# tirtho109/parallel_AMG

Hardware: AMD Instinct MI355X
Metric: V-cycle iters/sec + fine-SpMV HBM GB/s, 3D Poisson 128M dofs at 1/2/4/8 GPU (higher is better)
Workload: dtype f64; 1 GPU; poisson3d 512^3 fp64, SA-AMG V(1,1) weighted-Jacobi, 1 part(s); n=134217728, nnz_fine=937951232, levels=6, max_coarse=1000, parallelism=row-slab partition p1

## Files before the change

### include/pamg.h

```cpp
#ifndef PAMG_H
#define PAMG_H

#include <stdint.h>

#ifdef __cplusplus
extern "C" {
#endif

#define PAMG_OK 0
#define PAMG_E_ARG (-1)
#define PAMG_E_HIP (-2)
#define PAMG_E_RCCL (-3)
#define PAMG_E_OVERFLOW (-4)
#define PAMG_E_SETUP (-5)
#define PAMG_E_STATE (-6)
#define PAMG_E_NOMEM (-7)

typedef struct pamg_ctx pamg_ctx;
typedef struct pamg_plan pamg_plan;
typedef struct pamg_vec pamg_vec;
typedef struct pamg_mat pamg_mat;
typedef struct pamg_hier pamg_hier;
typedef struct pamg_hcsr pamg_hcsr;

// ... 42 lines not shown
int pamg_vec_download(pamg_ctx* ctx, const pamg_vec* v, double* own);
int pamg_vec_download_ghosts(pamg_ctx* ctx, const pamg_vec* v, double* ghost);
int pamg_vec_device_ptr(pamg_vec* v, double** dptr);
int pamg_vec_fill(pamg_ctx* ctx, pamg_vec* v, double value);
int pamg_vec_copy(pamg_ctx* ctx, const pamg_vec* src, pamg_vec* dst);
int pamg_vec_axpby(pamg_ctx* ctx, double a, const pamg_vec* x, double b, pamg_vec* y);
int pamg_vec_dot(pamg_ctx* ctx, const pamg_vec* x, const pamg_vec* y, double* out);
int pamg_vec_nrm2(pamg_ctx* ctx, const pamg_vec* x, double* out);
int pamg_exchange(pamg_ctx* ctx, const pamg_plan* plan, pamg_vec* x);
int pamg_exchange_begin(pamg_ctx* ctx, pamg_plan* plan, pamg_vec* x);
int pamg_exchange_end(pamg_ctx* ctx, pamg_plan* plan, pamg_vec* x);

int pamg_mat_upload(pamg_ctx* ctx, int64_t nrows, int64_t ncols_local, const int64_t* rowptr,
                    const void* col, int col_is_64, const double* val, int index_base,
                    const pamg_plan* col_plan, pamg_mat** out);
int pamg_mat_upload_perm(pamg_ctx* ctx, int64_t nrows, int64_t ncols_local, const int64_t* rowptr,
                         const void* col, int col_is_64, const double* val, int index_base,
                         const pamg_plan* col_plan, const int64_t* row_perm,
                         const int64_t* col_perm, pamg_mat** out);
int pamg_mat_destroy(pamg_mat* A);
int pamg_mat_info(const pamg_mat* A, int64_t* nrows, int64_t* ncols_local, int64_t* nnz);
int pamg_mat_stream_bytes(const pamg_mat* A, int64_t* bytes);
int pamg_mat_layout(const pamg_mat* A, int set, int out[10]);

int pamg_spmv(pamg_ctx* ctx, const pamg_mat* A, pamg_vec* x, pamg_vec* y);
int pamg_residual(pamg_ctx* ctx, const pamg_mat* A, pamg_vec* x, const pamg_vec* b,
                  pamg_vec* r, double* nrm2);
int pamg_jacobi(pamg_ctx* ctx, const pamg_mat* A, pamg_vec* x, const pamg_vec* b,
                pamg_vec* tmp, double omega, int nsweeps);
int pamg_jacobi_residual(pamg_ctx* ctx, const pamg_mat* A, pamg_vec* x, const pamg_vec* b,
                         pamg_vec* t, pamg_vec* r, double omega, int* fused);

int pamg_hier_create(pamg_ctx* ctx, int nlevels, pamg_mat* const* A, pamg_mat* const* P,
                     pamg_mat* const* R, const double* omega, int64_t n_coarse,
                     const double* ainv_colmajor, int rep_level, const int64_t* rep_offsets,
                     pamg_hier** out);
int pamg_hier_destroy(pamg_hier* H);
int pamg_hier_set_graph(pamg_hier* H, int enable);
int pamg_hier_set_sweeps(pamg_hier* H, int nu1, int nu2);
int pamg_hier_set_perm(pamg_hier* H, int64_t n, const int64_t* perm);
int pamg_hier_graph_state(const pamg_hier* H, int* enabled, int* captured, int* failed);
int pamg_vcycle(pamg_ctx* ctx, pamg_hier* H, pamg_vec* x, const pamg_vec* b, int ncycles,
                double* res_hist);
int pamg_vcycle_async(pamg_ctx* ctx, pamg_hier* H, pamg_vec* x, const pamg_vec* b, int ncycles);
int pamg_pcg(pamg_ctx* ctx, pamg_hier* H, pamg_vec* x, const pamg_vec* b, double rtol,
             int maxit, int* iters, double* res_hist);
// ... 51 lines not shown
```

### parallel_amg_amd/_lib.py

```python
from __future__ import annotations

import ctypes as C
import os

_HERE = os.path.dirname(os.path.abspath(__file__))
LIB_PATH = os.environ.get("PAMG_LIB") or os.path.join(_HERE, "libpamg.so")

PAMG_OK = 0
ERRORS = {-1: "PAMG_E_ARG", -2: "PAMG_E_HIP", -3: "PAMG_E_RCCL", -4: "PAMG_E_OVERFLOW",
          -5: "PAMG_E_SETUP", -6: "PAMG_E_STATE", -7: "PAMG_E_NOMEM"}


class PamgError(RuntimeError):
    def __init__(self, code, fn, msg):
        super().__init__(f"{fn} -> {ERRORS.get(code, code)}: {msg}")
        self.code = code


vp = C.c_void_p
i32, i64, dbl = C.c_int, C.c_int64, C.c_double
pvp = C.POINTER(C.c_void_p)
pi64 = C.POINTER(C.c_int64)
pdbl = C.POINTER(C.c_double)
pi32 = C.POINTER(C.c_int32)
# ... 27 lines not shown
    "pamg_plan_set_tag": [vp, i64],
    "pamg_plan_destroy": [vp],
    "pamg_vec_create": [vp, i64, i64, pvp],
    "pamg_vec_destroy": [vp],
    "pamg_vec_size": [vp, pi64, pi64],
    "pamg_vec_upload": [vp, vp, vp],
    "pamg_vec_download": [vp, vp, vp],
    "pamg_vec_download_ghosts": [vp, vp, vp],
    "pamg_vec_device_ptr": [vp, pvp],
    "pamg_vec_fill": [vp, vp, dbl],
    "pamg_vec_copy": [vp, vp, vp],
    "pamg_vec_axpby": [vp, dbl, vp, dbl, vp],
    "pamg_vec_dot": [vp, vp, vp, pdbl],
    "pamg_vec_nrm2": [vp, vp, pdbl],
    "pamg_exchange": [vp, vp, vp],
    "pamg_exchange_begin": [vp, vp, vp],
    "pamg_exchange_end": [vp, vp, vp],
    "pamg_mat_upload": [vp, i64, i64, vp, vp, i32, vp, i32, vp, pvp],
    "pamg_mat_upload_perm": [vp, i64, i64, vp, vp, i32, vp, i32, vp, vp, vp, pvp],
    "pamg_mat_destroy": [vp],
    "pamg_mat_info": [vp, pi64, pi64, pi64],
    "pamg_mat_stream_bytes": [vp, pi64],
    "pamg_mat_layout": [vp, i32, C.POINTER(C.c_int)],
    "pamg_spmv": [vp, vp, vp, vp],
    "pamg_residual": [vp, vp, vp, vp, vp, pdbl],
    "pamg_jacobi": [vp, vp, vp, vp, vp, dbl, i32],
    "pamg_jacobi_residual": [vp, vp, vp, vp, vp, vp, dbl, pi32],
    "pamg_hier_create": [vp, i32, vp, vp, vp, vp, i64, vp, i32, vp, pvp],
    "pamg_hier_destroy": [vp],
    "pamg_hier_set_graph": [vp, i32],
    "pamg_hier_set_sweeps": [vp, i32, i32],
    "pamg_hier_set_perm": [vp, i64, vp],
    "pamg_hier_graph_state": [vp, C.POINTER(C.c_int), C.POINTER(C.c_int), C.POINTER(C.c_int)],
    "pamg_vcycle": [vp, vp, vp, vp, i32, vp],
    "pamg_vcycle_async": [vp, vp, vp, vp, i32],
    "pamg_pcg": [vp, vp, vp, vp, dbl, i32, C.POINTER(C.c_int), vp],
    "pamg_hier_profile": [vp, i32],
    "pamg_hier_profile_read": [vp, vp],
    "pamg_bench_rowop": [vp, vp, i32, vp, vp, vp, dbl, i32, pdbl],
    "pamg_hier_bench_chain": [vp, vp, vp, i32, pdbl],
    "pamg_set_option": [C.c_char_p, i64],
    "pamg_get_option": [C.c_char_p, pi64],
    "pamg_hcsr_create": [i64, i64, i64, pvp],
    "pamg_hcsr_destroy": [vp],
    "pamg_hcsr_info": [vp, pi64, pi64, pi64],
    "pamg_hcsr_data": [vp, C.POINTER(pi64), C.POINTER(pi32), C.POINTER(pdbl)],
# ... 50 lines not shown
    for key, sym in (("hip", "hipStreamCreateWithFlags"), ("rccl", "ncclCommInitRank")):
        try:
            addr = C.cast(getattr(L, sym), C.c_void_p).value
        except AttributeError:
            continue
        info = _DlInfo()
        if addr and dladdr(addr, C.byref(info)) and info.dli_fname:
            out[key] = os.path.realpath(info.dli_fname.decode())
    return out


def call(name, *args):
    L = lib()
    rc = getattr(L, name)(*args)
    if rc != PAMG_OK:
        msg = L.pamg_last_error().decode(errors="replace")
        raise PamgError(rc, name, msg)
    return rc


def layout_of(M, part_set: int = 0) -> dict:
    out = (C.c_int * 10)()
    call("pamg_mat_layout", M.handle, part_set, out)
    return {"c24": bool(out[0]), "vd": bool(out[1]), "rl8": bool(out[2]), "cd": int(out[3]),
            "cd_offsets": int(out[4]), "tm": bool(out[5]), "tm_rs": int(out[6]),
            "tile_nnz": int(out[7]), "tiles": int(out[8]), "anchored": bool(out[9] & 1), "per_tile": bool(out[9] & 2),
            "x_stage": bool(out[9] & 4), "sym": bool(out[9] & 8), "sym_rows": 2 if out[9] & 16 else 1,
            "jr_fused": bool(out[9] & 32), "tm_vd": bool(out[9] & 64), "sym_vd": bool(out[9] & 128),
            "ell": bool(out[9] & 512), "pnc": bool(out[9] & 1024),
            "rpat": bool(out[9] & 2048), "pnc_compact": bool(out[9] & 4096),
            "ell_pair": bool(out[9] & 8192)}


def last_error() -> str:
    return lib().pamg_last_error().decode(errors="replace")


def ptr(a):
    return C.c_void_p(a.ctypes.data) if a is not None and a.size else None
```

### parallel_amg_amd/csrc/kernels.hip

```cpp

#include "pamg_device.h"

namespace pamg {
namespace {

__device__ __forceinline__ int wave_incl_scan(int v) {
    const int lane = threadIdx.x & 63, rl = lane & 15;
    int t;
    t = __builtin_amdgcn_mov_dpp(v, 0x111, 0xf, 0xf, false);
    if (rl >= 1) v += t;
    t = __builtin_amdgcn_mov_dpp(v, 0x112, 0xf, 0xf, false);
    if (rl >= 2) v += t;
    t = __builtin_amdgcn_mov_dpp(v, 0x114, 0xf, 0xf, false);
    if (rl >= 4) v += t;
    t = __builtin_amdgcn_mov_dpp(v, 0x118, 0xf, 0xf, false);
    if (rl >= 8) v += t;
    t = __builtin_amdgcn_mov_dpp(v, 0x142, 0xf, 0xf, false);
    if (lane & 16) v += t;
    t = __builtin_amdgcn_mov_dpp(v, 0x143, 0xf, 0xf, false);
    if (lane >= 32) v += t;
    return v;
}

template <int OP>
// ... 1477 lines not shown
            const bool ok = 4 * q + e < L;
            const double p = vv[e] * xv[e];
            const double t = s + p;
            s = ok ? t : s;
            if constexpr (OP == OP_JACOBI) dg = ok && of[e] == 0 ? vv[e] : dg;
        }
    }
    double out;
    if constexpr (OP == OP_SPMV) {
        out = s;
    } else if constexpr (OP == OP_RESID) {
        out = pb - s;
    } else if constexpr (OP == OP_JACOBI) {
        const double u = pb - s;
        const double v = omega * u;
        const double w = v / dg;
        out = px + w;
    } else {
        out = py + s;
    }
    if (in) y[i] = out;
}

template <int OP, int U>
__global__ __launch_bounds__(kEllGroup) void k_rows_rpat(int nrows, const int* __restrict__ gorder,
                                                         const int* __restrict__ anc, const uint8_t* __restrict__ pid,
                                                         const int2* __restrict__ pmeta, int npat,
                                                         const uint32_t* __restrict__ pent, int nent,
                                                         const double* __restrict__ vtab, int nval, int ngroups,
                                                         const double* __restrict__ x, const double* __restrict__ b,
                                                         double* __restrict__ y, double omega) {
    __shared__ uint32_t le[kRpatEnt];
    __shared__ int2 lm[kRpatMax];
    __shared__ double lv[256];
    const int per = (ngroups + 7) / 8;
    const int gi = (blockIdx.x & 7) * per + (blockIdx.x >> 3);
    if (gi >= ngroups) return;
    const int g = gorder ? gorder[gi] : gi;
    const int tid = threadIdx.x;
    const int i = g * kEllGroup + tid;
    const int ic = i < nrows ? i : nrows - 1;
    const int p = i < nrows ? (int)pid[i] : kRpatSkip;
    const int a = anc[ic];
    double pb = 0.0, px = 0.0, py = 0.0;
    if constexpr (OP == OP_RESID || OP == OP_JACOBI) pb = b[ic];
    if constexpr (OP == OP_JACOBI) px = x[ic];
// ... 525 lines not shown

template <int OP>
void launch_rpat(const pamg_mat& A, const double* x, const double* b, double* y, double omega, hipStream_t s) {
    const RpatSet& R = A.rpat;
    const int grid = (int)((R.ngroups + 7) / 8 * 8);
    auto go = [&](auto kern) {
        kern<<<grid, kEllGroup, 0, s>>>((int)A.nrows, R.d_gorder, R.d_anc, R.d_pid, R.d_pmeta, R.npat, R.d_pent, R.nent,
                                        R.d_vtab, R.nval, (int)R.ngroups, x, b, y, omega);
    };
    go(k_rows_rpat<OP, 8>);
}

template <int OP>
void launch_rows_op(const pamg_mat& A, const TileSet& ts, const double* x, const double* b,
                    double* y, double omega, hipStream_t s) {
    if (ts.sym) launch_sym<OP>(A, x, b, y, omega, s);
    if (ts.ell) {
        const EllSet& E = A.ell;
        const int grid = (int)((E.ngroups + 7) / 8 * 8);
        auto go = [&](auto kern) {
            kern<<<grid, kEllGroup, 0, s>>>((int)A.nrows, E.d_gorder, E.d_anc, E.d_smeta, E.d_ci, E.d_vi, E.d_len,
                                            E.d_gmeta, E.d_otab, E.d_vtab, (int)E.ngroups, x, b, y, omega);
        };
        if (E.d_anc) {
            if (E.paired) go(k_rows_ell<OP, true, true>);
            else go(k_rows_ell<OP, true, false>);
        } else {
            if (E.paired) go(k_rows_ell<OP, false, true>);
            else go(k_rows_ell<OP, false, false>);
        }
    }
    if (ts.pnc) launch_pnc<OP>(A, x, b, y, omega, s);
    if (ts.rpat) launch_rpat<OP>(A, x, b, y, omega, s);
    if (ts.n_short > 0) {
        if (ts.tile_nnz == 1024) launch_tile<OP, 1024>(A, ts, x, b, y, omega, s);
        else if (ts.tile_nnz == 4096) launch_tile<OP, 4096>(A, ts, x, b, y, omega, s);
        else launch_tile<OP, 2048>(A, ts, x, b, y, omega, s);
    }
    if (ts.n_long > 0)
        k_rows_long<OP><<<ts.n_long, kBlock, 0, s>>>(ts.d_long, A.d_rowptr, A.d_col, A.d_val, x,
                                                     b, y, omega);
}
}

void launch_sym_tb(const pamg_mat& A, const TbArgs& ta, hipStream_t s) {
    SymDia sd = A.sym;
    TbGeom& g = sd.tb;
// ... 106 lines not shown
```

### parallel_amg_amd/csrc/pamg_device.h

```cpp
#pragma once

#include <hip/hip_runtime.h>
#include <rccl/rccl.h>

#include <atomic>
#include <cstdint>
#include <array>
#include <mutex>
#include <vector>

#include "pamg_common.h"

namespace pamg {

constexpr int kBlock = 256;
constexpr int kTileRows = 256;

constexpr int kXsMaxClusters = 12;
constexpr int kTmSmallTab = 128;
constexpr int kXsCap = 1088;
constexpr int kXsIoff = 128;
constexpr int kXsGap = 48;
struct XStage {
    int ncl = 0, stride = 0, zix = -1, ncols = 0;
// ... 56 lines not shown
    int col_dict = 1;
    int tile_major = 1;
    int col_dict_tile = 1;
    int tm_tile_dicts = 1;
    int band_pct = 100;
    int band_pct_restrict = 50;
    int x_stage = 1;
    int col_dict_anchor = 1;
    int poison_ghosts = 0;
    int sym_dia = 1;
    int sym_rows = 2;
    int jr_fuse = 1;
    int symd_chunks = 2;
    int chain_store_x = 0;
    int tb_xfast = 1;
    int sym_zm = 1;
    int zm_chunks = 0;
    int ell = 1;
    int ell_min_rows = 65536;
    int ell_restrict = 1;
    int ell_yblock = 16;
    int rpat = 1;
    int ell_pair = 1;
    int pnc_compact = 1;
    int pnc = 1;
    int sym_vd = 1;
};

constexpr int kSymMaxU = 7;
constexpr int kSymVdMax = 64;
struct TbGeom {
    int nx = 0, ny = 0, nz = 0;
    int tiles_x = 0, tiles_y = 0;
    int zchunks = 1, zlen = 0;
    int zlo = 0, zhi = 0;
    int xfast = 0;
};
constexpr int kEllW = 64;
constexpr int kEllGroup = 256;
constexpr int kEllSkip = 255;
struct EllSet {
    int64_t nslices = 0, ngroups = 0;
    int2* d_smeta = nullptr;
    uint32_t* d_ci = nullptr;
    uint32_t* d_vi = nullptr;
    uint8_t* d_len = nullptr;
    int4* d_gmeta = nullptr;
    int* d_otab = nullptr;
    double* d_vtab = nullptr;
    int* d_anc = nullptr;
    int* d_gorder = nullptr;
    int64_t words = 0, otab_n = 0, vtab_n = 0;
    bool paired = false;
};

constexpr int kPncPatMax = 1024, kPncValMax = 128, kPncMaxLen = 7;
constexpr int kPncSkip = kPncPatMax - 1;
constexpr int kPncCombMax = 1024;
constexpr int kPncCombSkip = 0xffff;
struct PncSet {
    int nx = 0, ny = 0, nz = 0;
    int* d_anc = nullptr;
    uint2* d_rec = nullptr;
    uint16_t* d_cid = nullptr;
    uint64_t* d_pvals = nullptr;
    uint32_t* d_ptab = nullptr;
    double* d_vtab = nullptr;
    int npat = 0, nval = 0;
    int grid = 0;
};

constexpr int kRpatMax = 255, kRpatEnt = 4096, kRpatMaxLen = 128;
constexpr int kRpatSkip = 255;
struct RpatSet {
    int64_t ngroups = 0;
    int* d_anc = nullptr;
// ... 134 lines not shown
```

### parallel_amg_amd/csrc/runtime.hip

```cpp
#include <dlfcn.h>

#include <algorithm>
#include <array>
#include <atomic>
#include <functional>
#include <chrono>
#include <condition_variable>
#include <mutex>
#include <cstdio>
#include <cstdlib>
#include <cstring>
#include <map>
#include <memory>
#include <mutex>
#include <string>
#include <thread>
#include <vector>

#include "pamg_device.h"

using pamg::fail;

pamg::Options& pamg::options() {
    static Options o;
    return o;
}

#define HIPC(expr)                                                                    \
// ... 1108 lines not shown
            const int64_t gnx = gr[1], gny = gr[2], gM = gr[1] * gr[2];
            std::vector<int64_t> key(ng);
            par_for(ng, [&](int64_t a, int64_t b) {
                for (int64_t g = a; g < b; ++g) {
                    const int64_t c = anc[g * kEllGroup];
                    const int64_t y = (c / gnx) % gny, z = c / gM;
                    key[g] = ((y / yb) << 40) | (z << 20) | y;
                }
            });
            const int64_t per = (ng + 7) / 8;
            std::vector<int> order(ng);
            for (int64_t g = 0; g < ng; ++g) order[g] = (int)g;
            for (int64_t e = 0; e < 8; ++e) {
                const int64_t lo = std::min(ng, e * per), hi = std::min(ng, (e + 1) * per);
                std::stable_sort(order.begin() + lo, order.begin() + hi, [&](int p, int q) { return key[p] < key[q]; });
            }
            CHECK(dalloc(d_order, ng));
            CHECK(h2d(ctx, *d_order, order.data(), sizeof(int) * ng));
            break;
        }
    return PAMG_OK;
}

int build_ell(pamg_mat* A, const PtrVec& rp, const IdxVec& ci, const double* val,
              bool anchored, const std::vector<int>& inner) {
    using pamg::kEllGroup;
    using pamg::kEllSkip;
    using pamg::kEllW;
    const int64_t n = A->nrows;
    std::vector<char> in_set;
    if ((int64_t)inner.size() != n) {
        in_set.assign(n, 0);
        for (int i : inner) in_set[i] = 1;
    }
    auto member = [&](int64_t i) { return in_set.empty() || in_set[i]; };
    auto base_of = [&](int64_t i) -> int { return anchored ? (rp[i + 1] > rp[i] ? ci[rp[i]] : 0) : (int)i; };
    const int64_t ns = (n + kEllW - 1) / kEllW, ng = (n + kEllGroup - 1) / kEllGroup;
    std::vector<int> slen(ns, 0);
    std::atomic<bool> ok{true};
    par_for(ns, [&](int64_t a, int64_t b) {
        for (int64_t q = a; q < b; ++q) {
            int m = 0;
            for (int64_t i = q * kEllW; i < std::min(n, (q + 1) * kEllW); ++i)
                if (member(i)) m = std::max<int>(m, (int)(rp[i + 1] - rp[i]));
            if (m >= kEllSkip) ok = false;
            slen[q] = m;
        }
    });
    if (!ok) return PAMG_OK;
    std::vector<int2> smeta(ns);
    int64_t words = 0;
    for (int64_t q = 0; q < ns; ++q) {
        smeta[q] = make_int2((int)words, slen[q]);
        words += (int64_t)kEllW * ((slen[q] + 3) / 4);
        if (words >= INT32_MAX) return PAMG_OK;
    }
    std::vector<std::vector<int>> goff(ng);
    std::vector<std::vector<uint64_t>> gval(ng);
    std::vector<uint32_t> cw(words + 1, 0u), vw;
    std::vector<uint8_t> len(n + kVecPad, 0);
    bool paired = pamg::options().ell_pair != 0;
    if (paired) {
        std::atomic<bool> fits{true};
        par_for(ng, [&](int64_t a, int64_t b) {
            constexpr int kSlots = 1024;
            std::vector<int> pid(kSlots), pstamp(kSlots, -1), pkey_o(kSlots);
            std::vector<uint64_t> pkey_v(kSlots);
            std::vector<int> o;
            std::vector<uint64_t> v;
            for (int64_t g = a; g < b && fits; ++g) {
                const int stamp = (int)(g - a);
                o.clear();
                v.clear();
                const int64_t r1 = std::min(n, (g + 1) * kEllGroup);
                for (int64_t i = g * kEllGroup; i < r1 && fits; ++i) {
                    if (!member(i)) {
                        len[i] = (uint8_t)kEllSkip;
                        continue;
// ... 481 lines not shown
    R = pamg::RpatSet{};
}

void free_pnc(pamg::PncSet& P) {
    dfree(P.d_anc);
    dfree(P.d_rec);
    dfree(P.d_cid);
    dfree(P.d_pvals);
    dfree(P.d_ptab);
    dfree(P.d_vtab);
    P = pamg::PncSet{};
}

void free_ell(pamg::EllSet& E) {
    dfree(E.d_gorder);
    dfree(E.d_smeta);
    dfree(E.d_ci);
    dfree(E.d_vi);
    dfree(E.d_len);
    dfree(E.d_gmeta);
    dfree(E.d_otab);
    dfree(E.d_vtab);
    dfree(E.d_anc);
    E = pamg::EllSet{};
}

void free_tiles(pamg::TileSet& ts) {
    dfree(ts.d_short);
    dfree(ts.d_long);
    dfree(ts.d_base);
    dfree(ts.d_vtab);
    dfree(ts.d_ctab);
    ts.cd = ts.ctab_n = 0;
    dfree(ts.d_tm_val);
    dfree(ts.d_tm_cidx);
    dfree(ts.d_tm_clo);
    dfree(ts.d_tm_chi);
    dfree(ts.d_tm_rlen);
    dfree(ts.d_tm_anc);
    dfree(ts.d_tm_vidx);
    dfree(ts.d_tm_vtab);
    ts.tm_vt = 0;
    dfree(ts.d_abase);
    ts.anc = ts.pt = ts.xs = false;
    ts.tm = false;
    ts.tm_rs = 0;
// ... 1253 lines not shown
        CHECK(build_col_dicts(A.get(), rp, ci, t_in, t_bd, &idx8));
        tr.mark("col dicts");
        CHECK(build_tile_major(A.get(), n_own_cols, rp, ci, val, t_in, t_bd, lo, hi, idx8));
        tr.mark("tile-major");
    }
    if (A->interior.rl8 || A->boundary.rl8) {
        std::vector<uint8_t> rl(nrows + kVecPad, 0);
        par_for(nrows, [&](int64_t a, int64_t b) {
            for (int64_t i = a; i < b; ++i) rl[i] = (uint8_t)std::min<int64_t>(255, rp[i + 1] - rp[i]);
        });
        CHECK(dalloc(&A->d_rlen, nrows + kVecPad));
        CHECK(h2d(ctx, A->d_rlen, rl.data(), rl.size()));
    }
    if (!vidx.empty()) {
        CHECK(dalloc(&A->d_vidx, (int64_t)vidx.size()));
        CHECK(h2d(ctx, A->d_vidx, vidx.data(), vidx.size()));
    }
    A->stream_bytes = 4;
    if (A->interior.sym)
        A->stream_bytes += A->sym.vd_n ? nrows + (int64_t)A->sym.vd_n * (8 * (A->sym.nu + 1) + 4)
                                       : nrows * (A->sym.mask_bytes + 8 + 8 * (int64_t)A->sym.nu);
    if (A->interior.ell)
        A->stream_bytes += (A->ell.paired ? 4 : 8) * A->ell.words + nrows + 8 * A->ell.nslices + 16 * A->ell.ngroups + 4 * A->ell.otab_n +
                           8 * A->ell.vtab_n + (A->ell.d_anc ? 4 * nrows : 0);
    if (A->interior.pnc)
        A->stream_bytes += (A->pnc.d_cid ? 6 : 12) * nrows + (A->pnc.d_cid ? 12 : 4) * A->pnc.npat + 8 * A->pnc.nval;
    if (A->interior.rpat) A->stream_bytes += 5 * nrows + 8 * A->rpat.npat + 4 * A->rpat.nent + 8 * A->rpat.nval;
    for (const pamg::TileSet* t : {&A->interior, &A->boundary}) {
        if (t->sym || t->ell || t->pnc || t->rpat) continue;
        const int64_t ns = t->n_short, nz = t->nnz_short;
        int64_t b = 8 * (int64_t)t->n_long + 12 * t->nnz_long;
        const bool base = t->c24 && !t->cd;
        if (t->tm) {
            const int64_t tn = t->tile_nnz;
            const int64_t rowb = t->tm_rs;
            const int64_t valb = t->tm_vt ? tn + 8 * (int64_t)t->tm_vt : 8 * tn;
            b += ns * (rowb * (t->anc ? 5 : 1) + valb + (t->cd ? t->cd * tn / 8 : 3 * tn) + 16 + (base ? 4 : 0)) +
                 (t->cd ? 4 * t->ctab_n * (t->pt ? ns : 1) : 0);
        } else {
            b += (t->rl8 ? 1 : 4) * t->rows_short;
            b += t->cd ? (t->cd * nz + 7) / 8 + 4 * t->ctab_n * (t->pt ? ns : 1) : (t->c24 ? 3 : 4) * nz;
            if (t->pt && t->anc) b += 2 * t->rows_short + 4 * ns;
            b += t->vd ? nz / 2 + 128 * ns : 8 * nz;
            b += (16 + (base ? 4 : 0)) * ns;
        }
        A->stream_bytes += b;
    }
// ... 126 lines not shown
    out[5] = t.tm;
    out[6] = t.tm_rs;
    out[7] = t.tile_nnz;
    out[8] = t.n_short;
    out[9] = (t.anc ? 1 : 0) | (t.pt ? 2 : 0) | (t.xs ? 4 : 0) | (t.sym ? 8 : 0) | (t.sym && A->sym.rpl == 2 ? 16 : 0) |
             (t.sym && (A->sym.tb_ok || A->sym.tb_part) ? 32 : 0) | (t.tm && t.tm_vt ? 64 : 0) |
             (t.sym && A->sym.vd_n ? 128 : 0) | (t.ell ? 512 : 0) | (t.pnc ? 1024 : 0) | (t.rpat ? 2048 : 0) |
             (t.pnc && A->pnc.d_cid ? 4096 : 0) | (t.ell && A->ell.paired ? 8192 : 0);
    if (t.ell) out[8] = (int)A->ell.ngroups;
    if (t.rpat) {
        out[3] = A->rpat.nval;
        out[4] = A->rpat.npat;
        out[8] = (int)A->rpat.ngroups;
    }
    if (t.pnc) {
        out[3] = A->pnc.nval;
        out[4] = A->pnc.npat;
        out[8] = A->pnc.grid;
    }
    if (t.sym) {
        out[4] = A->sym.nu;
        out[8] = A->sym.nbands * 8 * A->sym.eighth;
    }
    return PAMG_OK;
}

static int check_vec_for(const pamg_mat* A, const pamg_vec* x, const char* who) {
    const int64_t need_ghost = A->plan ? A->plan->n_ghost : 0;
    const int64_t own = A->plan ? A->plan->n_own : A->ncols;
    if (x->n_own != own || x->n_ghost < need_ghost)
        return fail(PAMG_E_ARG, "%s: input vector (%lld own, %lld ghost) does not fit the matrix columns (%lld own, %lld ghost)",
                    who, (long long)x->n_own, (long long)x->n_ghost, (long long)own, (long long)need_ghost);
    return PAMG_OK;
}

int pamg_spmv(pamg_ctx* ctx, const pamg_mat* A, pamg_vec* x, pamg_vec* y) {
    if (!ctx || !A || !x || !y) return fail(PAMG_E_ARG, "spmv: NULL");
    CHECK(check_vec_for(A, x, "spmv"));
    if (y->n_own != A->nrows) return fail(PAMG_E_ARG, "spmv: output size mismatch");
    if (x == y) return fail(PAMG_E_ARG, "spmv: x and y must differ");
    CHECK(set_device(ctx));
    CHECK(apply(ctx, A, pamg::OP_SPMV, x->d, nullptr, y->d, 0.0));
    HIPC(hipStreamSynchronize(ctx->s_comp));
    return PAMG_OK;
}

// ... 584 lines not shown
    else if (k == "value_dict" && value >= 0 && value <= 2) o.value_dict = (int)value;
    else if (k == "col_dict" && (value == 0 || value == 1)) o.col_dict = (int)value;
    else if (k == "tile_major" && value >= 0 && value <= 2) o.tile_major = (int)value;
    else if (k == "col_dict_anchor" && (value == 0 || value == 1)) o.col_dict_anchor = (int)value;
    else if (k == "col_dict_tile" && (value == 0 || value == 1)) o.col_dict_tile = (int)value;
    else if (k == "x_stage" && (value == 0 || value == 1)) o.x_stage = (int)value;
    else if (k == "band_pct" && value >= 1 && value <= 10000) o.band_pct = (int)value;
    else if (k == "band_pct_restrict" && value >= 1 && value <= 10000) o.band_pct_restrict = (int)value;
    else if (k == "long_tiles_min" && value >= 1 && value <= 255) o.long_tiles_min = (int)value;
    else if (k == "tm_tile_dicts" && (value == 0 || value == 1)) o.tm_tile_dicts = (int)value;
    else if (k == "sym_dia" && (value == 0 || value == 1)) o.sym_dia = (int)value;
    else if (k == "sym_rows" && (value == 1 || value == 2)) o.sym_rows = (int)value;
    else if (k == "jr_fuse" && (value == 0 || value == 1)) o.jr_fuse = (int)value;
    else if (k == "sym_vd" && (value == 0 || value == 1)) o.sym_vd = (int)value;
    else if (k == "symd_chunks" && (value == 1 || value == 2 || value == 4)) o.symd_chunks = (int)value;
    else if (k == "sym_zm" && (value == 0 || value == 1)) o.sym_zm = (int)value;
    else if (k == "tb_xfast" && (value == 0 || value == 1)) o.tb_xfast = (int)value;
    else if (k == "ell" && (value == 0 || value == 1)) o.ell = (int)value;
    else if (k == "ell_restrict" && (value == 0 || value == 1)) o.ell_restrict = (int)value;
    else if (k == "pnc" && (value == 0 || value == 1)) o.pnc = (int)value;
    else if (k == "rpat" && (value == 0 || value == 1)) o.rpat = (int)value;
    else if (k == "pnc_compact" && (value == 0 || value == 1)) o.pnc_compact = (int)value;
    else if (k == "ell_pair" && (value == 0 || value == 1)) o.ell_pair = (int)value;
    else if (k == "ell_yblock" && value >= 0 && value <= 65536) o.ell_yblock = (int)value;
    else if (k == "ell_min_rows" && value >= 0 && value <= INT32_MAX) o.ell_min_rows = (int)value;
    else if (k == "zm_chunks" && value >= 0 && value <= 4096) o.zm_chunks = (int)value;
    else if (k == "chain_store_x" && (value == 0 || value == 1)) o.chain_store_x = (int)value;
    else return fail(PAMG_E_ARG, "set_option: unknown key or bad value: %s=%lld", key, (long long)value);
    return PAMG_OK;
}

int pamg_get_option(const char* key, int64_t* value) {
    if (!key || !value) return fail(PAMG_E_ARG, "get_option: bad args");
    const auto& o = pamg::options();
    const std::string k(key);
    if (k == "tile_nnz") *value = o.tile_nnz;
    else if (k == "tile_order") *value = o.tile_order;
    else if (k == "long_tiles") *value = o.long_tiles;
    else if (k == "row_len8") *value = o.row_len8;
    else if (k == "poison_ghosts") *value = o.poison_ghosts;
    else if (k == "col24") *value = o.col24;
    else if (k == "value_dict") *value = o.value_dict;
    else if (k == "col_dict") *value = o.col_dict;
    else if (k == "tile_major") *value = o.tile_major;
    else if (k == "col_dict_anchor") *value = o.col_dict_anchor;
    else if (k == "col_dict_tile") *value = o.col_dict_tile;
    else if (k == "x_stage") *value = o.x_stage;
    else if (k == "band_pct") *value = o.band_pct;
    else if (k == "band_pct_restrict") *value = o.band_pct_restrict;
    else if (k == "long_tiles_min") *value = o.long_tiles_min;
    else if (k == "tm_tile_dicts") *value = o.tm_tile_dicts;
    else if (k == "sym_dia") *value = o.sym_dia;
    else if (k == "sym_rows") *value = o.sym_rows;
    else if (k == "jr_fuse") *value = o.jr_fuse;
    else if (k == "sym_vd") *value = o.sym_vd;
    else if (k == "symd_chunks") *value = o.symd_chunks;
    else if (k == "sym_zm") *value = o.sym_zm;
    else if (k == "tb_xfast") *value = o.tb_xfast;
    else if (k == "ell") *value = o.ell;
    else if (k == "ell_restrict") *value = o.ell_restrict;
    else if (k == "pnc") *value = o.pnc;
    else if (k == "rpat") *value = o.rpat;
    else if (k == "pnc_compact") *value = o.pnc_compact;
    else if (k == "ell_pair") *value = o.ell_pair;
    else if (k == "ell_yblock") *value = o.ell_yblock;
    else if (k == "ell_min_rows") *value = o.ell_min_rows;
    else if (k == "zm_chunks") *value = o.zm_chunks;
    else if (k == "chain_store_x") *value = o.chain_store_x;
    else return fail(PAMG_E_ARG, "get_option: unknown key %s", key);
    return PAMG_OK;
}

int pamg_hier_bench_chain(pamg_hier* H, pamg_vec* x, const pamg_vec* b, int reps, double* avg_ms) {
    if (!H || !x || !b || reps < 1 || !avg_ms) return fail(PAMG_E_ARG, "hier_bench_chain: bad args");
    if (!pipe_ok(H, 2, false)) return fail(PAMG_E_STATE, "hier_bench_chain: the hierarchy does not run the cross-cycle pipeline");
    pamg_ctx* ctx = H->ctx;
    CHECK(check_vec_for(H->A[0], x, "hier_bench_chain"));
    CHECK(set_device(ctx));
    if (!H->u0) {
        const int64_t n = H->nown[0] + (H->A[0]->plan ? H->A[0]->plan->n_ghost : 0) + kVecPad;
        CHECK(dalloc(&H->u0, n));
        CHECK(dzero(H->ctx, H->u0, sizeof(double) * n));
    }
    hipEvent_t e0, e1;
    HIPC(hipEventCreate(&e0));
    HIPC(hipEventCreate(&e1));
    hipStream_t s = ctx->s_comp;
// ... 75 lines not shown
```

Baseline: 218.9 V-cycles/s.

## Add windowed ELL kernel staging x into LDS via async global_load_lds

Adds an ELL variant that groups four row slices by shared (offset,value) pairs and column coupling, then stages the contiguous x window each group touches into LDS with global_load_lds before the row sweep. Rows then read x from LDS using 16-bit local offsets instead of gathering from global memory. The aim is to cut redundant and uncoalesced x gathers in the ELL row kernels (spmv, residual, jacobi, prolong), which mostly hit coarse levels. In exchange it adds a heavy host-side grouping pass, extra metadata streams (chunks, lof, dpos), and LDS pressure that may lower occupancy; it is gated on window size and share thresholds.

```diff
diff --git a/include/pamg.h b/include/pamg.h
--- a/include/pamg.h
+++ b/include/pamg.h
@@ -88,6 +88,7 @@
 int pamg_mat_info(const pamg_mat* A, int64_t* nrows, int64_t* ncols_local, int64_t* nnz);
 int pamg_mat_stream_bytes(const pamg_mat* A, int64_t* bytes);
 int pamg_mat_layout(const pamg_mat* A, int set, int out[10]);
+int pamg_mat_ell_window(const pamg_mat* A, int out[16]);
 
 int pamg_spmv(pamg_ctx* ctx, const pamg_mat* A, pamg_vec* x, pamg_vec* y);
 int pamg_residual(pamg_ctx* ctx, const pamg_mat* A, pamg_vec* x, const pamg_vec* b,
diff --git a/parallel_amg_amd/_lib.py b/parallel_amg_amd/_lib.py
--- a/parallel_amg_amd/_lib.py
+++ b/parallel_amg_amd/_lib.py
@@ -73,6 +73,7 @@
     "pamg_mat_info": [vp, pi64, pi64, pi64],
     "pamg_mat_stream_bytes": [vp, pi64],
     "pamg_mat_layout": [vp, i32, C.POINTER(C.c_int)],
+    "pamg_mat_ell_window": [vp, C.POINTER(C.c_int)],
     "pamg_spmv": [vp, vp, vp, vp],
     "pamg_residual": [vp, vp, vp, vp, vp, pdbl],
     "pamg_jacobi": [vp, vp, vp, vp, vp, dbl, i32],
@@ -169,7 +170,16 @@
 def layout_of(M, part_set: int = 0) -> dict:
     out = (C.c_int * 10)()
     call("pamg_mat_layout", M.handle, part_set, out)
-    return {"c24": bool(out[0]), "vd": bool(out[1]), "rl8": bool(out[2]), "cd": int(out[3]),
+    win = (C.c_int * 16)()
+    if part_set == 0:
+        call("pamg_mat_ell_window", M.handle, win)
+    return {"ell_xwin": bool(win[0]), "ell_xwin_groups": int(win[1]), "ell_gather_groups": int(win[2]),
+            "ell_xwin_max_window": int(win[3]), "ell_xwin_noncontig_groups": int(win[4]),
+            "ell_xwin_max_pairs": int(win[5]), "ell_xwin_max_chunks": int(win[6]),
+            "ell_xwin_census": {"groups": int(win[7]), "full_groups": int(win[13]), "window_mean": int(win[8]),
+                                "window_p95": int(win[9]), "runs_mean": int(win[10]), "runs_max": int(win[11]),
+                                "pairs_mean": int(win[12])},
+            "c24": bool(out[0]), "vd": bool(out[1]), "rl8": bool(out[2]), "cd": int(out[3]),
             "cd_offsets": int(out[4]), "tm": bool(out[5]), "tm_rs": int(out[6]),
             "tile_nnz": int(out[7]), "tiles": int(out[8]), "anchored": bool(out[9] & 1), "per_tile": bool(out[9] & 2),
             "x_stage": bool(out[9] & 4), "sym": bool(out[9] & 8), "sym_rows": 2 if out[9] & 16 else 1,
diff --git a/parallel_amg_amd/csrc/kernels.hip b/parallel_amg_amd/csrc/kernels.hip
--- a/parallel_amg_amd/csrc/kernels.hip
+++ b/parallel_amg_amd/csrc/kernels.hip
@@ -1523,6 +1523,139 @@
     if (in) y[i] = out;
 }
 
+template <bool WIN>
+__device__ __forceinline__ void ellw_dword(uint32_t cq, int q, int L, int lane, int row,
+                                           const double* __restrict__ lv, const uint16_t* __restrict__ lof,
+                                           const double* __restrict__ lx, const int* __restrict__ lo,
+                                           const double* __restrict__ x, double& s) {
+    int of[4];
+    double vv[4], xv[4];
+#pragma unroll
+    for (int e = 0; e < 4; ++e) {
+        const uint32_t p = (cq >> (8 * e)) & 255u;
+        vv[e] = lv[p];
+        if constexpr (WIN) of[e] = (int)lof[p] - 64 + lane;
+        else of[e] = lo[p];
+    }
+#pragma unroll
+    for (int e = 0; e < 4; ++e) {
+        if constexpr (WIN) xv[e] = lx[4 * q + e < L ? of[e] : lane];
+        else xv[e] = x[4 * q + e < L ? row + of[e] : row];
+    }
+#pragma unroll
+    for (int e = 0; e < 4; ++e) {
+        const bool ok = 4 * q + e < L;
+        const double p = vv[e] * xv[e];
+        const double t = s + p;
+        s = ok ? t : s;
+    }
+}
+
+constexpr int kEllwPre = 12;
+__device__ __forceinline__ void ellw_load(uint32_t (&cq)[kEllwPre], const uint32_t* __restrict__ cw, int first, int nq,
+                                          int q0) {
+#pragma unroll
+    for (int e = 0; e < kEllwPre; ++e) cq[e] = cw[nq > 0 ? first + min(q0 + e, nq - 1) * kEllW : 0];
+}
+
+template <int OP>
+__global__ __launch_bounds__(kEllGroup) void k_rows_ellw(int nrows, const int4* __restrict__ gslices,
+                                                         const int2* __restrict__ smeta, const uint32_t* __restrict__ cw,
+                                                         const uint8_t* __restrict__ len, const uint8_t* __restrict__ dpos,
+                                                         const int4* __restrict__ gmeta, const int* __restrict__ otab,
+                                                         const double* __restrict__ vtab, const int4* __restrict__ wmeta, const int2* __restrict__ chunks,
+                                                         const uint16_t* __restrict__ lofs, int win, int gather_all,
+                                                         int ngroups, const double* __restrict__ x,
+                                                         const double* __restrict__ b, double* __restrict__ y,
+                                                         double omega) {
+    extern __shared__ double ellw_lds[];
+    double* lx = ellw_lds;
+    double* lv = ellw_lds + win;
+    uint16_t* lof = reinterpret_cast<uint16_t*>(lv + 256);
+    const int per = (ngroups + 7) / 8;
+    const int g = (blockIdx.x & 7) * per + (blockIdx.x >> 3);
+    if (g >= ngroups) return;
+    const int tid = threadIdx.x, lane = tid & 63;
+    const int w = __builtin_amdgcn_readfirstlane(tid >> 6);
+    const int4 gm = gmeta[g], wm = wmeta[g], gs = gslices[g];
+    const int np = gm.y;
+    const bool windowed = wm.y > 0 && !gather_all;
+    const double vtv = vtab[gm.x + (tid < np ? tid : 0)];
+    const uint32_t* __restrict__ l32 = reinterpret_cast<const uint32_t*>(lofs + wm.z);
+    const uint32_t la = l32[windowed && tid < 2 * np ? tid : 0], lb = l32[windowed && tid + 256 < 2 * np ? tid + 256 : 0];
+    const int2 cmv = chunks[wm.x + (w + 4 * lane < wm.y ? w + 4 * lane : 0)];
+    const int slice = w == 0 ? gs.x : w == 1 ? gs.y : w == 2 ? gs.z : gs.w;
+    const int i = slice * kEllW + lane;
+    const bool in = slice >= 0 && i < nrows;
+    const int ic = in ? i : 0;
+    const int L = in ? (int)len[ic] : 0;
+    const int2 sm = smeta[slice >= 0 ? slice : 0];
+    const int nq = slice >= 0 ? (sm.y + 3) >> 2 : 0;
+    const uint32_t* __restrict__ cp = cw + sm.x + lane;
+    double pb = 0.0, px = 0.0, py = 0.0;
+    if constexpr (OP == OP_RESID || OP == OP_JACOBI) pb = b[ic];
+    if constexpr (OP == OP_JACOBI) px = x[ic];
+    if constexpr (OP == OP_PROLONG) py = y[ic];
+    uint32_t dkw = 0u;
+    int dk = 255;
+    if constexpr (OP == OP_JACOBI) {
+        dk = in ? (int)dpos[ic] : 255;
+        dkw = cw[dk != 255 ? sm.x + lane + (dk >> 2) * kEllW : 0];
+    }
+    double s = 0.0;
+    if (windowed) {
+        uint32_t cq[kEllwPre];
+        ellw_load(cq, cw, sm.x + lane, nq, 0);
+        for (int k = 0; w + 4 * k < wm.y; ++k) {
+            const int col = __builtin_amdgcn_readlane(cmv.x, k), sc = __builtin_amdgcn_readlane(cmv.y, k);
+            if (lane < (sc >> 16))
+                __builtin_amdgcn_global_load_lds(
+                    (const __attribute__((address_space(1))) void*)(x + col + 2 * lane),
+                    (__attribute__((address_space(3))) void*)(lx + (sc & 0xffff)), 16, 0, 0);
+        }
+        if (tid < np) lv[tid] = vtv;
+        if (tid < 2 * np) reinterpret_cast<uint32_t*>(lof)[tid] = la;
+        if (tid + 256 < 2 * np) reinterpret_cast<uint32_t*>(lof)[tid + 256] = lb;
+        __syncthreads();
+        for (int q0 = 0; q0 < nq; q0 += kEllwPre) {
+            if (q0 > 0) ellw_load(cq, cw, sm.x + lane, nq, q0);
+#pragma unroll
+            for (int e = 0; e < kEllwPre; ++e)
+                if (q0 + e < nq)
+                    ellw_dword<true>(cq[e], q0 + e, L, lane, ic, lv, lof + w * np, lx, nullptr, x, s);
+        }
+    } else {
+        int* lo = reinterpret_cast<int*>(lx);
+        const int otv = otab[gm.x + (tid < np ? tid : 0)];
+        if (tid < np) {
+            lo[tid] = otv;
+            lv[tid] = vtv;
+        }
+        __syncthreads();
+        uint32_t c4 = nq > 0 ? cp[0] : 0u;
+        for (int q = 0; q < nq; ++q) {
+            const uint32_t cq = c4;
+            if (q + 1 < nq) c4 = cp[(q + 1) * kEllW];
+            ellw_dword<false>(cq, q, L, lane, ic, lv, nullptr, nullptr, lo, x, s);
+        }
+    }
+    double out;
+    if constexpr (OP == OP_SPMV) {
+        out = s;
+    } else if constexpr (OP == OP_RESID) {
+        out = pb - s;
+    } else if constexpr (OP == OP_JACOBI) {
+        const double u = pb - s;
+        const double v = omega * u;
+        const double dg = dk != 255 ? lv[(dkw >> (8 * (dk & 3))) & 255u] : 0.0;
+        const double wq = v / dg;
+        out = px + wq;
+    } else {
+        out = py + s;
+    }
+    if (in) y[i] = out;
+}
+
 template <int OP, int U>
 __global__ __launch_bounds__(kEllGroup) void k_rows_rpat(int nrows, const int* __restrict__ gorder,
                                                          const int* __restrict__ anc, const uint8_t* __restrict__ pid,
@@ -2094,7 +2227,14 @@
             kern<<<grid, kEllGroup, 0, s>>>((int)A.nrows, E.d_gorder, E.d_anc, E.d_smeta, E.d_ci, E.d_vi, E.d_len,
                                             E.d_gmeta, E.d_otab, E.d_vtab, (int)E.ngroups, x, b, y, omega);
         };
-        if (E.d_anc) {
+        if (E.win) {
+            const int win = std::max(E.max_window, 128);
+            const size_t lds = sizeof(double) * (size_t)(win + 256) + sizeof(uint16_t) * 4 * 256;
+            k_rows_ellw<OP><<<grid, kEllGroup, lds, s>>>(
+                (int)A.nrows, E.d_gslices, E.d_smeta, E.d_ci, E.d_len, E.d_dpos, E.d_gmeta, E.d_otab, E.d_vtab, E.d_wmeta,
+                E.d_chunks, E.d_lof, win, (reinterpret_cast<uintptr_t>(x) & 15) != 0 ? 1 : 0, (int)E.ngroups, x, b, y,
+                omega);
+        } else if (E.d_anc) {
             if (E.paired) go(k_rows_ell<OP, true, true>);
             else go(k_rows_ell<OP, true, false>);
         } else {
diff --git a/parallel_amg_amd/csrc/pamg_device.h b/parallel_amg_amd/csrc/pamg_device.h
--- a/parallel_amg_amd/csrc/pamg_device.h
+++ b/parallel_amg_amd/csrc/pamg_device.h
@@ -102,6 +102,8 @@
     int ell_yblock = 16;
     int rpat = 1;
     int ell_pair = 1;
+    int ell_xwin = 1;
+    int ell_xwin_max = 7168;
     int pnc_compact = 1;
     int pnc = 1;
     int sym_vd = 1;
@@ -119,6 +121,12 @@
 constexpr int kEllW = 64;
 constexpr int kEllGroup = 256;
 constexpr int kEllSkip = 255;
+constexpr int kEllWinCap = 7168;
+constexpr int kEllWinChunks = 256;
+constexpr int kEllLdsPerCu = 160 * 1024;
+constexpr int kEllWinKeep = 85;
+constexpr int kEllWinMinShare = 50;
+constexpr int kEllWinMinRatio100 = 150;
 struct EllSet {
     int64_t nslices = 0, ngroups = 0;
     int2* d_smeta = nullptr;
@@ -132,6 +140,16 @@
     int* d_gorder = nullptr;
     int64_t words = 0, otab_n = 0, vtab_n = 0;
     bool paired = false;
+    bool win = false;
+    int4* d_gslices = nullptr;
+    int4* d_wmeta = nullptr;
+    int2* d_chunks = nullptr;
+    uint16_t* d_lof = nullptr;
+    uint8_t* d_dpos = nullptr;
+    int64_t nchunks = 0, lof_n = 0;
+    int win_groups = 0, gather_groups = 0, noncontig_groups = 0;
+    int max_window = 0, max_pairs = 0, max_chunks = 0;
+    int mean_window = 0, p95_window = 0, mean_runs = 0, max_runs = 0, mean_pairs = 0, full_groups = 0;
 };
 
 constexpr int kPncPatMax = 1024, kPncValMax = 128, kPncMaxLen = 7;
diff --git a/parallel_amg_amd/csrc/runtime.hip b/parallel_amg_amd/csrc/runtime.hip
--- a/parallel_amg_amd/csrc/runtime.hip
+++ b/parallel_amg_amd/csrc/runtime.hip
@@ -4,6 +4,7 @@
 #include <array>
 #include <atomic>
 #include <functional>
+#include <iterator>
 #include <chrono>
 #include <condition_variable>
 #include <mutex>
@@ -1158,6 +1159,319 @@
     return PAMG_OK;
 }
 
+int build_ell_xwin(pamg_mat* A, const PtrVec& rp, const IdxVec& ci, const double* val,
+                   const std::vector<int2>& smeta, int64_t words) {
+    using pamg::kEllW;
+    const int64_t n = A->nrows, ns = (n + kEllW - 1) / kEllW;
+    const int cap = std::min(pamg::options().ell_xwin_max, pamg::kEllWinCap);
+    auto pair_key = [](int off, uint64_t u) {
+        uint64_t h = (u ^ (u >> 29)) * 0x9E3779B97F4A7C15ull + (uint64_t)(uint32_t)off * 0xC2B2AE3D27D4EB4Full;
+        return h ^ (h >> 32);
+    };
+    std::vector<std::vector<uint64_t>> spair(ns);
+    std::vector<std::vector<std::pair<int, int>>> scoup(ns);
+    std::atomic<bool> ok{true};
+    par_for(ns, [&](int64_t a, int64_t b) {
+        std::vector<uint64_t> h;
+        std::vector<int> t;
+        for (int64_t q = a; q < b && ok; ++q) {
+            h.clear();
+            t.clear();
+            for (int64_t i = q * kEllW; i < std::min(n, (q + 1) * kEllW); ++i)
+                for (int64_t k = rp[i]; k < rp[i + 1]; ++k) {
+                    uint64_t u;
+                    std::memcpy(&u, &val[k], 8);
+                    h.push_back(pair_key(ci[k] - (int)i, u));
+                    t.push_back(ci[k] / kEllW);
+                }
+            std::sort(h.begin(), h.end());
+            h.erase(std::unique(h.begin(), h.end()), h.end());
+            if (h.size() > 256) ok = false;
+            spair[q] = h;
+            std::sort(t.begin(), t.end());
+            for (size_t e = 0; e < t.size();) {
+                size_t f = e;
+                while (f < t.size() && t[f] == t[e]) ++f;
+                if (t[e] != q) scoup[q].push_back({t[e], (int)(f - e)});
+                e = f;
+            }
+        }
+    });
+    if (!ok) return PAMG_OK;
+    std::vector<std::array<int, 4>> grp;
+    grp.reserve(ns / 4 + 1);
+    {
+        std::vector<char> done(ns, 0);
+        std::vector<int> score(ns, 0), touched, cand;
+        std::vector<uint64_t> un, tmp;
+        auto couple = [&](int q) {
+            for (const auto& c : scoup[q])
+                if (!done[c.first]) {
+                    if (score[c.first] == 0) touched.push_back(c.first);
+                    score[c.first] += c.second;
+                }
+        };
+        for (int64_t first = 0; first < ns; ++first) {
+            if (done[first]) continue;
+            std::array<int, 4> g = {(int)first, -1, -1, -1};
+            done[first] = 1;
+            un = spair[first];
+            touched.clear();
+            couple((int)first);
+            for (int m = 1; m < 4; ++m) {
+                cand.clear();
+                for (int t : touched)
+                    if (!done[t]) cand.push_back(t);
+                if (cand.empty()) {
+                    int64_t t = first + 1;
+                    while (t < ns && done[t]) ++t;
+                    if (t < ns) cand.push_back((int)t);
+                }
+                const size_t top = std::min<size_t>(6, cand.size());
+                std::partial_sort(cand.begin(), cand.begin() + top, cand.end(), [&](int p, int q) {
+                    return score[p] != score[q] ? score[p] > score[q] : p < q;
+                });
+                int take = -1;
+                for (size_t c = 0; c < top && take < 0; ++c) {
+                    tmp.clear();
+                    std::set_union(un.begin(), un.end(), spair[cand[c]].begin(), spair[cand[c]].end(),
+                                   std::back_inserter(tmp));
+                    if (tmp.size() <= 256) take = cand[c];
+                }
+                if (take < 0) break;
+                un.swap(tmp);
+                g[m] = take;
+                done[take] = 1;
+                couple(take);
+            }
+            for (int t : touched) score[t] = 0;
+            grp.push_back(g);
+        }
+    }
+    std::vector<std::vector<std::pair<int, int>>>().swap(scoup);
+    std::vector<std::vector<uint64_t>>().swap(spair);
+    const int64_t ng = (int64_t)grp.size();
+    std::vector<std::vector<int>> goff(ng);
+    std::vector<std::vector<uint64_t>> gval(ng);
+    std::vector<std::vector<int2>> gchunk(ng);
+    std::vector<std::vector<uint16_t>> glof(ng);
+    std::vector<int> gwin(ng, 0), gruns(ng, 0);
+    std::vector<int64_t> gnnz(ng, 0);
+    std::vector<uint32_t> cw(words + 1, 0u);
+    std::vector<uint8_t> len(n + kVecPad, 0), dpos(n + kVecPad, (uint8_t)255);
+    par_for(ng, [&](int64_t a, int64_t b) {
+        constexpr int kSlots = 1024;
+        std::vector<int> pid(kSlots), pstamp(kSlots, -1), pkey_o(kSlots);
+        std::vector<uint64_t> pkey_v(kSlots);
+        std::vector<int> o, lmin(4 * 256), lmax(4 * 256);
+        std::vector<uint64_t> v;
+        std::vector<std::array<int, 2>> rng;
+        std::vector<std::array<int, 3>> runs;
+        for (int64_t g = a; g < b && ok; ++g) {
+            const int stamp = (int)(g - a);
+            o.clear();
+            v.clear();
+            for (int w = 0; w < 4 && ok; ++w) {
+                const int64_t q = grp[g][w];
+                if (q < 0) continue;
+                for (int64_t i = q * kEllW; i < std::min(n, (q + 1) * kEllW) && ok; ++i) {
+                    len[i] = (uint8_t)(rp[i + 1] - rp[i]);
+                    gnnz[g] += rp[i + 1] - rp[i];
+                    const int lane = (int)(i % kEllW);
+                    for (int64_t k = rp[i]; k < rp[i + 1]; ++k) {
+                        const int kk = (int)(k - rp[i]);
+                        const int off = ci[k] - (int)i;
+                        if (off == 0) dpos[i] = (uint8_t)kk;
+                        uint64_t u;
+                        std::memcpy(&u, &val[k], 8);
+                        uint32_t h = (uint32_t)((((uint64_t)(uint32_t)off * 0x9E3779B1u) ^ u ^ (u >> 29)) *
+                                                0x9E3779B97F4A7C15ull >> 54);
+                        while (pstamp[h] == stamp && (pkey_o[h] != off || pkey_v[h] != u)) h = (h + 1) & (kSlots - 1);
+                        if (pstamp[h] != stamp) {
+                            if (o.size() == 256) {
+                                ok = false;
+                                break;
+                            }
+                            pstamp[h] = stamp;
+                            pkey_o[h] = off;
+                            pkey_v[h] = u;
+                            pid[h] = (int)o.size();
+                            for (int x = 0; x < 4; ++x) {
+                                lmin[x * 256 + pid[h]] = kEllW;
+                                lmax[x * 256 + pid[h]] = -1;
+                            }
+                            o.push_back(off);
+                            v.push_back(u);
+                        }
+                        const int p = pid[h];
+                        lmin[w * 256 + p] = std::min(lmin[w * 256 + p], lane);
+                        lmax[w * 256 + p] = std::max(lmax[w * 256 + p], lane);
+                        const int64_t wd = smeta[q].x + (int64_t)(kk / 4) * kEllW + lane;
+                        cw[wd] |= (uint32_t)p << (8 * (kk % 4));
+                    }
+                }
+            }
+            if (!ok) break;
+            goff[g] = o;
+            gval[g] = v;
+            const int np = (int)o.size();
+            rng.clear();
+            for (int w = 0; w < 4; ++w)
+                for (int p = 0; p < np; ++p)
+                    if (grp[g][w] >= 0 && lmax[w * 256 + p] >= 0) {
+                        const int c0 = grp[g][w] * kEllW + o[p];
+                        rng.push_back({c0 + lmin[w * 256 + p], c0 + lmax[w * 256 + p]});
+                    }
+            std::sort(rng.begin(), rng.end());
+            runs.clear();
+            for (const auto& r : rng) {
+                const int s = r[0] & ~1, e = (r[1] + 2) & ~1;
+                if (!runs.empty() && s <= runs.back()[1] + 16) runs.back()[1] = std::max(runs.back()[1], e);
+                else runs.push_back({s, e, 0});
+            }
+            int slots = 0, nch = 0;
+            for (auto& r : runs) {
+                r[2] = slots;
+                slots += r[1] - r[0];
+                nch += (r[1] - r[0] + 127) / 128;
+            }
+            if (slots == 0 || slots > cap || nch > pamg::kEllWinChunks) continue;
+            if (runs.front()[0] < 0 || runs.back()[1] > ((int)A->ncols + 1)) continue;
+            gwin[g] = slots;
+            gruns[g] = (int)runs.size();
+            for (const auto& r : runs)
+                for (int c = r[0]; c < r[1]; c += 128)
+                    gchunk[g].push_back(make_int2(c, (r[2] + c - r[0]) | (std::min(128, r[1] - c) / 2) << 16));
+            glof[g].assign((size_t)4 * np, (uint16_t)64);
+            for (int w = 0; w < 4; ++w)
+                for (int p = 0; p < np; ++p) {
+                    uint16_t word = 64;
+                    if (grp[g][w] >= 0 && lmax[w * 256 + p] >= 0) {
+                        const int c0 = grp[g][w] * kEllW + o[p], c = c0 + lmin[w * 256 + p];
+                        size_t r = 0;
+                        while (r + 1 < runs.size() && runs[r + 1][0] <= c) ++r;
+                        word = (uint16_t)(runs[r][2] + c0 - runs[r][0] + 64);
+                    }
+                    glof[g][(size_t)w * np + p] = word;
+                }
+        }
+    });
+    if (!ok) return PAMG_OK;
+    {
+        int64_t have = 0;
+        for (int64_t g = 0; g < ng; ++g) have += gwin[g] > 0;
+        for (int k = 8; k >= 2 && have > 0; --k) {
+            const int fit = ((pamg::kEllLdsPerCu / k - 2048) / 8 - 256) & ~1;
+            int64_t keep = 0;
+            for (int64_t g = 0; g < ng; ++g) keep += gwin[g] > 0 && gwin[g] <= fit;
+            if (keep * 100 < pamg::kEllWinKeep * have) continue;
+            for (int64_t g = 0; g < ng; ++g)
+                if (gwin[g] > fit) {
+                    gwin[g] = 0;
+                    gchunk[g].clear();
+                    glof[g].clear();
+                }
+            break;
+        }
+    }
+    pamg::EllSet& E = A->ell;
+    int64_t win_nnz = 0, win_slots = 0, win_runs = 0, win_pairs = 0;
+    for (int64_t g = 0; g < ng; ++g) {
+        E.max_pairs = std::max(E.max_pairs, (int)goff[g].size());
+        bool contig = true;
+        for (int w = 1; w < 4; ++w) contig = contig && (grp[g][w] < 0 || grp[g][w] == grp[g][0] + w);
+        if (gwin[g] > 0) {
+            ++E.win_groups;
+            win_nnz += gnnz[g];
+            win_slots += gwin[g];
+            E.max_window = std::max(E.max_window, gwin[g]);
+            E.max_chunks = std::max(E.max_chunks, (int)gchunk[g].size());
+            if (!contig) ++E.noncontig_groups;
+            win_runs += gruns[g];
+            win_pairs += (int64_t)goff[g].size();
+            E.max_runs = std::max(E.max_runs, gruns[g]);
+            if (grp[g][3] >= 0) ++E.full_groups;
+        } else {
+            ++E.gather_groups;
+        }
+    }
+    if ((int64_t)E.win_groups * 100 < pamg::kEllWinMinShare * ng || win_nnz * 100 < pamg::kEllWinMinRatio100 * win_slots) {
+        E = pamg::EllSet{};
+        return PAMG_OK;
+    }
+    {
+        std::vector<int> ws;
+        for (int64_t g = 0; g < ng; ++g)
+            if (gwin[g] > 0) ws.push_back(gwin[g]);
+        std::sort(ws.begin(), ws.end());
+        E.p95_window = ws[(ws.size() - 1) * 95 / 100];
+        E.mean_window = (int)(win_slots / E.win_groups);
+        E.mean_runs = (int)(win_runs / E.win_groups);
+        E.mean_pairs = (int)(win_pairs / E.win_groups);
+    }
+    std::vector<int4> gmeta(ng), wmeta(ng), gsl(ng);
+    int64_t on = 0, cn = 0, ln = 0;
+    for (int64_t g = 0; g < ng; ++g) {
+        const int np = (int)goff[g].size();
+        gmeta[g] = make_int4((int)on, np, (int)on, np);
+        wmeta[g] = make_int4((int)cn, (int)gchunk[g].size(), (int)ln, gwin[g]);
+        gsl[g] = make_int4(grp[g][0], grp[g][1], grp[g][2], grp[g][3]);
+        on += np;
+        cn += (int64_t)gchunk[g].size();
+        ln += (int64_t)glof[g].size();
+    }
+    if (ln >= INT32_MAX || cn >= INT32_MAX) {
+        E = pamg::EllSet{};
+        return PAMG_OK;
+    }
+    std::vector<int> otab(on + 1, 0);
+    std::vector<double> vtab(on + 1, 0.0);
+    std::vector<int2> chunks(cn + 1, make_int2(0, 0));
+    std::vector<uint16_t> lof(ln + 2, (uint16_t)0);
+    par_for(ng, [&](int64_t a, int64_t b) {
+        for (int64_t g = a; g < b; ++g) {
+            std::copy(goff[g].begin(), goff[g].end(), otab.begin() + gmeta[g].x);
+            for (size_t e = 0; e < gval[g].size(); ++e) std::memcpy(&vtab[gmeta[g].x + e], &gval[g][e], 8);
+            std::copy(gchunk[g].begin(), gchunk[g].end(), chunks.begin() + wmeta[g].x);
+            std::copy(glof[g].begin(), glof[g].end(), lof.begin() + wmeta[g].z);
+        }
+    });
+    pamg_ctx* ctx = A->ctx;
+    E.nslices = ns;
+    E.ngroups = ng;
+    E.words = words;
+    E.otab_n = on;
+    E.vtab_n = on;
+    E.paired = true;
+    E.win = true;
+    E.nchunks = cn;
+    E.lof_n = ln;
+    CHECK(dalloc(&E.d_smeta, ns));
+    CHECK(dalloc(&E.d_ci, words + 1));
+    CHECK(dalloc(&E.d_len, n + kVecPad));
+    CHECK(dalloc(&E.d_gmeta, ng));
+    CHECK(dalloc(&E.d_otab, on + 1));
+    CHECK(dalloc(&E.d_vtab, on + 1));
+    CHECK(dalloc(&E.d_gslices, ng));
+    CHECK(dalloc(&E.d_wmeta, ng));
+    CHECK(dalloc(&E.d_chunks, cn + 1));
+    CHECK(dalloc(&E.d_lof, ln + 2));
+    CHECK(dalloc(&E.d_dpos, n + kVecPad));
+    CHECK(h2d(ctx, E.d_dpos, dpos.data(), dpos.size()));
+    CHECK(h2d(ctx, E.d_smeta, smeta.data(), sizeof(int2) * ns));
+    CHECK(h2d(ctx, E.d_ci, cw.data(), sizeof(uint32_t) * (words + 1)));
+    CHECK(h2d(ctx, E.d_len, len.data(), len.size()));
+    CHECK(h2d(ctx, E.d_gmeta, gmeta.data(), sizeof(int4) * ng));
+    CHECK(h2d(ctx, E.d_otab, otab.data(), sizeof(int) * (on + 1)));
+    CHECK(h2d(ctx, E.d_vtab, vtab.data(), sizeof(double) * (on + 1)));
+    CHECK(h2d(ctx, E.d_gslices, gsl.data(), sizeof(int4) * ng));
+    CHECK(h2d(ctx, E.d_wmeta, wmeta.data(), sizeof(int4) * ng));
+    CHECK(h2d(ctx, E.d_chunks, chunks.data(), sizeof(int2) * (cn + 1)));
+    CHECK(h2d(ctx, E.d_lof, lof.data(), sizeof(uint16_t) * (ln + 2)));
+    A->interior.ell = true;
+    return PAMG_OK;
+}
+
 int build_ell(pamg_mat* A, const PtrVec& rp, const IdxVec& ci, const double* val,
               bool anchored, const std::vector<int>& inner) {
     using pamg::kEllGroup;
@@ -1190,6 +1504,10 @@
         smeta[q] = make_int2((int)words, slen[q]);
         words += (int64_t)kEllW * ((slen[q] + 3) / 4);
         if (words >= INT32_MAX) return PAMG_OK;
+    }
+    if (!anchored && in_set.empty() && !A->plan && pamg::options().ell_pair && pamg::options().ell_xwin) {
+        CHECK(build_ell_xwin(A, rp, ci, val, smeta, words));
+        if (A->interior.ell) return PAMG_OK;
     }
     std::vector<std::vector<int>> goff(ng);
     std::vector<std::vector<uint64_t>> gval(ng);
@@ -1717,6 +2035,11 @@
     dfree(E.d_otab);
     dfree(E.d_vtab);
     dfree(E.d_anc);
+    dfree(E.d_gslices);
+    dfree(E.d_wmeta);
+    dfree(E.d_chunks);
+    dfree(E.d_lof);
+    dfree(E.d_dpos);
     E = pamg::EllSet{};
 }
 
@@ -3016,7 +3339,8 @@
                                        : nrows * (A->sym.mask_bytes + 8 + 8 * (int64_t)A->sym.nu);
     if (A->interior.ell)
         A->stream_bytes += (A->ell.paired ? 4 : 8) * A->ell.words + nrows + 8 * A->ell.nslices + 16 * A->ell.ngroups + 4 * A->ell.otab_n +
-                           8 * A->ell.vtab_n + (A->ell.d_anc ? 4 * nrows : 0);
+                           8 * A->ell.vtab_n + (A->ell.d_anc ? 4 * nrows : 0) +
+                           (A->ell.win ? 32 * A->ell.ngroups + 8 * A->ell.nchunks + 2 * A->ell.lof_n + nrows : 0);
     if (A->interior.pnc)
         A->stream_bytes += (A->pnc.d_cid ? 6 : 12) * nrows + (A->pnc.d_cid ? 12 : 4) * A->pnc.npat + 8 * A->pnc.nval;
     if (A->interior.rpat) A->stream_bytes += 5 * nrows + 8 * A->rpat.npat + 4 * A->rpat.nent + 8 * A->rpat.nval;
@@ -3189,6 +3513,28 @@
         out[4] = A->sym.nu;
         out[8] = A->sym.nbands * 8 * A->sym.eighth;
     }
+    return PAMG_OK;
+}
+
+int pamg_mat_ell_window(const pamg_mat* A, int out[16]) {
+    if (!A || !out) return fail(PAMG_E_ARG, "mat_ell_window: bad args");
+    const pamg::EllSet& E = A->ell;
+    const bool w = A->interior.ell && E.win;
+    out[0] = w ? 1 : 0;
+    out[1] = w ? E.win_groups : 0;
+    out[2] = w ? E.gather_groups : 0;
+    out[3] = w ? E.max_window : 0;
+    out[4] = w ? E.noncontig_groups : 0;
+    out[5] = w ? E.max_pairs : 0;
+    out[6] = w ? E.max_chunks : 0;
+    out[7] = w ? (int)E.ngroups : 0;
+    out[8] = w ? E.mean_window : 0;
+    out[9] = w ? E.p95_window : 0;
+    out[10] = w ? E.mean_runs : 0;
+    out[11] = w ? E.max_runs : 0;
+    out[12] = w ? E.mean_pairs : 0;
+    out[13] = w ? E.full_groups : 0;
+    out[14] = out[15] = 0;
     return PAMG_OK;
 }
 
@@ -3819,6 +4165,8 @@
     else if (k == "rpat" && (value == 0 || value == 1)) o.rpat = (int)value;
     else if (k == "pnc_compact" && (value == 0 || value == 1)) o.pnc_compact = (int)value;
     else if (k == "ell_pair" && (value == 0 || value == 1)) o.ell_pair = (int)value;
+    else if (k == "ell_xwin" && (value == 0 || value == 1)) o.ell_xwin = (int)value;
+    else if (k == "ell_xwin_max" && value >= 2 && value <= pamg::kEllWinCap) o.ell_xwin_max = (int)value;
     else if (k == "ell_yblock" && value >= 0 && value <= 65536) o.ell_yblock = (int)value;
     else if (k == "ell_min_rows" && value >= 0 && value <= INT32_MAX) o.ell_min_rows = (int)value;
     else if (k == "zm_chunks" && value >= 0 && value <= 4096) o.zm_chunks = (int)value;
@@ -3860,6 +4208,8 @@
     else if (k == "rpat") *value = o.rpat;
     else if (k == "pnc_compact") *value = o.pnc_compact;
     else if (k == "ell_pair") *value = o.ell_pair;
+    else if (k == "ell_xwin") *value = o.ell_xwin;
+    else if (k == "ell_xwin_max") *value = o.ell_xwin_max;
     else if (k == "ell_yblock") *value = o.ell_yblock;
     else if (k == "ell_min_rows") *value = o.ell_min_rows;
     else if (k == "zm_chunks") *value = o.zm_chunks;
```

Result: faster. 224.6 V-cycles/s (median of 6 runs) (+2.6%).
